# Livioni/OmniVGGT-official

Measured on AMD Instinct MI355X. Metric: frames/sec (518^2, S views) aggregator hot path, higher is better.
Workload: dtype bf16

## Files before the change

omnivggt-official_amd/csrc/ovg_gemm.hip:

```cpp
#include "ovg_common.h"
#include <mutex>
#include <type_traits>
#include <utility>
#include <vector>

namespace {

constexpr int BM = 128, BN = 128;

#ifdef OVG_GEMM_TIMELINE
__device__ unsigned long long* g_tl_buf = nullptr;
__device__ int g_tl_stagger = 0;
OVG_DEV void tl_mark(int slot) {
  if ((threadIdx.x & 63) != 0 || g_tl_buf == nullptr) return;
  const int wave = threadIdx.x >> 6, last = (blockDim.x >> 6) - 1;
  if (wave != 0 && wave != last) return;
  unsigned long long* row = g_tl_buf + (size_t)blockIdx.x * 16 + (wave == 0 ? 0 : 8);
  row[slot] = wall_clock64();
  if (slot == 0) { row[4] = __builtin_amdgcn_s_getreg((31 << 11) | 4); row[5] = __builtin_amdgcn_s_getreg((31 << 11) | 20); row[6] = clock64(); }
  if (slot == 3) row[7] = clock64();
}
OVG_DEV void tl_stagger() {
  if (g_tl_stagger <= 0 || blockIdx.x >= 256) return;
  const unsigned long long until = wall_clock64() + (unsigned long long)(((blockIdx.x >> 3) & 7) * g_tl_stagger);
  while (wall_clock64() < until) __builtin_amdgcn_s_sleep(16);
}
#else
OVG_DEV void tl_mark(int) {}
OVG_DEV void tl_stagger() {}
#endif

OVG_DEV float gelu_erf(float x) { return 0.5f * x * (1.0f + erff(x * 0.70710678118654752440f)); }
OVG_DEV void gelu_poly16(f32x4 (&v)[4]) {
  constexpr float c[13] = {1.413637876e-01f, -7.029628064e-02f, 5.152052248e-02f, -4.044260701e-02f, 3.144217031e-02f, -2.326865498e-02f,
                           1.640218381e-02f, -1.116433345e-02f, 6.410491046e-03f, -2.685581490e-03f, 1.722817794e-03f, -1.613262584e-03f,
                           6.087207876e-04f};
  f32x4 xc[4], u[4], r[4];
#pragma unroll
  for (int nt = 0; nt < 4; ++nt) {
#pragma unroll
    for (int i = 0; i < 4; ++i) xc[nt][i] = __builtin_amdgcn_fmed3f(v[nt][i], -5.0f, 5.0f);
    u[nt] = xc[nt] * xc[nt] * 0.08f - 1.0f;
    r[nt] = u[nt] * c[12] + c[11];
  }
#pragma unroll
  for (int k = 10; k >= 0; --k) {
#pragma unroll
    for (int nt = 0; nt < 4; ++nt) r[nt] = r[nt] * u[nt] + c[k];
  }
#pragma unroll
  for (int nt = 0; nt < 4; ++nt) v[nt] = v[nt] * (xc[nt] * r[nt] + 0.5f);
}

OVG_DEV void tile_coords(int lid, int mtiles, int ntiles_gm, int& tm, int& tn) {
  const int ntiles = ntiles_gm & 0xffff, GM = (ntiles_gm >> 16) & 0xff;
  if (GM == 0) { tm = lid / ntiles; tn = lid - tm * ntiles; return; }
  const int per_group = GM * ntiles;
  const int grp = lid / per_group, rem = lid - grp * per_group;
  const int m_first = grp * GM;
  const int gsz = (mtiles - m_first) < GM ? (mtiles - m_first) : GM;
  tm = m_first + rem % gsz;
  tn = rem / gsz;
}

template <typename T, bool SWAP = false, bool X3 = false>
OVG_DEV void gemm_mainloop(const T* __restrict__ X, int64_t ldx, const T* __restrict__ W, int64_t ldw,
                           int M, int N, int K, int m0, int n0, unsigned char* lds, f32x4 (&acc)[4][4],
                           const T* __restrict__ Xlo = nullptr, const T* __restrict__ Wlo = nullptr) {
  constexpr int BKB = 128;
  unsigned char* Ws = lds;
  unsigned char* Xs = lds + BN * BKB;
  const int tid = threadIdx.x, lane = tid & 63, wave = tid >> 6;
  const int wn = wave >> 1, wm = wave & 1;
  const int g = lane >> 4, lr = lane & 15;

  const unsigned char* xg[4];
  const unsigned char* wg[4];
  int soff[4];
#pragma unroll
  for (int i = 0; i < 4; ++i) {
    const int row = (tid >> 3) + 32 * i, ch = tid & 7;
    int xr = m0 + row; xr = xr < M ? xr : M - 1;
    int wr = n0 + row; wr = wr < N ? wr : N - 1;
    xg[i] = reinterpret_cast<const unsigned char*>(X + (int64_t)xr * ldx) + ch * 16;
    wg[i] = reinterpret_cast<const unsigned char*>(W + (int64_t)wr * ldw) + ch * 16;
// ... 59 lines not shown
        a[t] = *reinterpret_cast<const u32x4*>(Ws + wrow + t * 16 * 128 + coff);
        b[t] = *reinterpret_cast<const u32x4*>(Xs + xrow + t * 16 * 128 + coff);
      }
#pragma unroll
      for (int nt = 0; nt < 4; ++nt)
#pragma unroll
        for (int mt = 0; mt < 4; ++mt) {
          if constexpr (SWAP) TT<T>::mma(acc[nt][mt], b[mt], a[nt]);
          else TT<T>::mma(acc[nt][mt], a[nt], b[mt]);
        }
    }
    __syncthreads();
    if (more) {
#pragma unroll
      for (int i = 0; i < 4; ++i) {
        *reinterpret_cast<u32x4*>(Xs + soff[i]) = rx[i];
        *reinterpret_cast<u32x4*>(Ws + soff[i]) = rw[i];
      }
      __syncthreads();
    }
  }
}

template <typename T, int EPI, bool OUT_F32, int MT, bool INJECT, bool X3 = false>
OVG_DEV void linear_epilogue_impl(const ovg_linear_params& p, const f32x4 (&acc)[4][MT], const int m_w0, const int n_w0) {
  const int M = (int)p.M, N = (int)p.N;
  const int lane = threadIdx.x & 63, g = lane >> 4, lr = lane & 15;
  const int ncol = n_w0 + 4 * g;
  f32x4 bias[4], gam[4];
  if (p.bias != nullptr) {
#pragma unroll
    for (int nt = 0; nt < 4; ++nt) bias[nt] = *reinterpret_cast<const f32x4*>(p.bias + ncol + nt * 16);
  } else {
#pragma unroll
    for (int nt = 0; nt < 4; ++nt) bias[nt] = f32x4{0.f, 0.f, 0.f, 0.f};
  }
  if constexpr (EPI == OVG_EPI_RES) {
#pragma unroll
    for (int nt = 0; nt < 4; ++nt) gam[nt] = *reinterpret_cast<const f32x4*>(p.gamma + ncol + nt * 16);
  }
  constexpr bool kRowLoads = (EPI == OVG_EPI_RES || EPI == OVG_EPI_PATCH);
  constexpr int AH = !kRowLoads ? 0 : (MT == 8 ? 1 : 0);
  constexpr int NS = AH + 1;
  const FastDiv div_p0(EPI == OVG_EPI_PATCH ? (int)p.p0 : 1), div_per(INJECT ? (int)p.inj_period : 1);
  f32x4 ex[NS][4], inj[NS][4];
  float on[NS];
  int64_t orow_s[NS];
  auto fetch = [&](int mt, f32x4 (&exs)[4], f32x4 (&injs)[4], float& ons, int64_t& orow) {
    const int m = m_w0 + mt * 16 + lr;
    const int mc = m < M ? m : M - 1;
    orow = mc;
    ons = 0.f;
    if constexpr (EPI == OVG_EPI_PATCH) {
      int vw, t;
      div_p0.divmod(mc, vw, t);
      orow = (int64_t)vw * p.p1 + p.row_off + t;
      const float* trow = p.table + (int64_t)(t + 1) * N + ncol;
#pragma unroll
// ... 57 lines not shown
          store4_hilo(static_cast<f16_t*>(p.y) + off, static_cast<f16_t*>(p.y_lo) + off, v[nt][0], v[nt][1], v[nt][2], v[nt][3]);
        } else {
          store4<T>(static_cast<T*>(p.y) + orow * p.ldy + ncol + nt * 16, v[nt][0], v[nt][1], v[nt][2], v[nt][3]);
        }
      }
    }
  }
}

template <typename T> OVG_DEV void stage16_put4(unsigned char* img, int row, int col, float a, float b, float c, float d) {
  const int chunk = col >> 3, half = (col >> 2) & 1;
  store4<T>(reinterpret_cast<T*>(img + row * 128 + ((chunk ^ (row & 7)) << 4) + half * 8), a, b, c, d);
}
OVG_DEV u32x4 stage16_get(const unsigned char* img, int row, int chunk) {
  return *reinterpret_cast<const u32x4*>(img + row * 128 + ((chunk ^ (row & 7)) << 4));
}
OVG_DEV void stage32_put4(unsigned char* img, int row, int col, const f32x4 v) {
  *reinterpret_cast<f32x4*>(img + row * 256 + (((col >> 2) ^ (row & 15)) << 4)) = v;
}
OVG_DEV f32x4 stage32_get(const unsigned char* img, int row, int chunk) {
  return *reinterpret_cast<const f32x4*>(img + row * 256 + ((chunk ^ (row & 15)) << 4));
}

template <typename T, int EPI, int MT>
OVG_DEV void linear_epilogue_staged(const ovg_linear_params& p, const f32x4 (&acc)[4][MT], const int m_w0, const int n_w0, unsigned char* img) {
  const int M = (int)p.M;
  const int lane = threadIdx.x & 63, g = lane >> 4, lr = lane & 15;
  const int ncol = n_w0 + 4 * g;
  f32x4 bias[4];
  if (p.bias != nullptr) {
#pragma unroll
    for (int nt = 0; nt < 4; ++nt) bias[nt] = *reinterpret_cast<const f32x4*>(p.bias + ncol + nt * 16);
  } else {
#pragma unroll
    for (int nt = 0; nt < 4; ++nt) bias[nt] = f32x4{0.f, 0.f, 0.f, 0.f};
  }
  if constexpr (EPI == OVG_EPI_RES) {
    constexpr int HR = 8 * MT, HB = MT / 2, NI = HR / 4;
    f32x4 gam[4];
#pragma unroll
    for (int nt = 0; nt < 4; ++nt) {
      gam[nt] = *reinterpret_cast<const f32x4*>(p.gamma + ncol + nt * 16);
      bias[nt] = gam[nt] * bias[nt];
    }
    const int prow = lane >> 4, pch = lane & 15;
#pragma unroll
    for (int half = 0; half < 2; ++half) {
      f32x4 res[NI];
#pragma unroll
      for (int i = 0; i < NI; ++i) {
        int m = m_w0 + half * HR + i * 4 + prow;
        m = m < M ? m : M - 1;
        res[i] = *reinterpret_cast<const f32x4*>(p.res + (int64_t)m * p.ldres + n_w0 + pch * 4);
      }
#pragma unroll
      for (int ml = 0; ml < HB; ++ml)
#pragma unroll
        for (int nt = 0; nt < 4; ++nt) stage32_put4(img, ml * 16 + lr, nt * 16 + 4 * g, gam[nt] * acc[nt][half * HB + ml] + bias[nt]);
#pragma unroll
// ... 21 lines not shown
          for (int nt = 0; nt < 4; ++nt)
#pragma unroll
            for (int r = 0; r < 4; ++r) v[nt][r] = fminf(v[nt][r], 65504.0f);
        }
      }
#pragma unroll
      for (int nt = 0; nt < 4; ++nt) stage16_put4<T>(img, mt * 16 + lr, nt * 16 + 4 * g, v[nt][0], v[nt][1], v[nt][2], v[nt][3]);
    }
    const int prow = lane >> 3, pch = lane & 7;
#pragma unroll
    for (int i0 = 0; i0 < 2 * MT; i0 += 4) {
      u32x4 t[4];
#pragma unroll
      for (int j = 0; j < 4; ++j) t[j] = stage16_get(img, (i0 + j) * 8 + prow, pch);
#pragma unroll
      for (int j = 0; j < 4; ++j) {
        const int m = m_w0 + (i0 + j) * 8 + prow;
        if (m < M) *reinterpret_cast<u32x4*>(static_cast<T*>(p.y) + (int64_t)m * p.ldy + n_w0 + pch * 8) = t[j];
      }
    }
  }
}

template <typename T, int EPI, bool OUT_F32, int MT, bool X3 = false>
OVG_DEV void linear_epilogue(const ovg_linear_params& p, const f32x4 (&acc)[4][MT], const int m_w0, const int n_w0) {
  if constexpr (EPI == OVG_EPI_RES) {
    if (p.inject != nullptr) { linear_epilogue_impl<T, EPI, OUT_F32, MT, true, X3>(p, acc, m_w0, n_w0); return; }
  }
  linear_epilogue_impl<T, EPI, OUT_F32, MT, false, X3>(p, acc, m_w0, n_w0);
}

template <typename T, int EPI, bool OUT_F32, int MT, bool X3 = false>
OVG_DEV void linear_epilogue_auto(const ovg_linear_params& p, const f32x4 (&acc)[4][MT], const int m_w0, const int n_w0, unsigned char* img) {
  if constexpr (sizeof(T) == 2) {
    if constexpr ((EPI == OVG_EPI_STORE || EPI == OVG_EPI_GELU) && !OUT_F32 && !X3) {
      if (((p.ldy * (int64_t)sizeof(T)) & 15) == 0) { linear_epilogue_staged<T, EPI, MT>(p, acc, m_w0, n_w0, img); return; }
    }
    if constexpr (EPI == OVG_EPI_RES) {
      bool inj_here = false;
      if (p.inject != nullptr) {
        const int rem = m_w0 % (int)p.inj_period;
        inj_here = rem == 0 || (int)p.inj_period - rem < 16 * MT;
      }
      if (!inj_here) { linear_epilogue_staged<T, EPI, MT>(p, acc, m_w0, n_w0, img); return; }
    }
  }
  linear_epilogue<T, EPI, OUT_F32, MT, X3>(p, acc, m_w0, n_w0);
}


template <typename T, int EPI, bool OUT_F32, bool X3 = false>
__global__ __launch_bounds__(256, 2) void linear_kernel(ovg_linear_params p, int ntiles_n) {
  __shared__ __attribute__((aligned(16))) unsigned char lds[2 * 128 * 128];
  const int M = (int)p.M, N = (int)p.N, K = (int)p.K;
  int tm, tn;
  tl_stagger();
  tl_mark(0);
  tile_coords(xcd_remap(blockIdx.x, gridDim.x), (M + BM - 1) / BM, ntiles_n, tm, tn);
  const int m0 = tm * BM, n0 = tn * BN;
  f32x4 acc[4][4];
  gemm_mainloop<T, false, X3>(static_cast<const T*>(p.x), p.ldx, static_cast<const T*>(p.w), p.ldw, M, N, K, m0, n0, lds, acc,
                              static_cast<const T*>(p.x_lo), static_cast<const T*>(p.w_lo));
  tl_mark(2);
  const int wave = __builtin_amdgcn_readfirstlane(threadIdx.x >> 6);
  linear_epilogue_auto<T, EPI, OUT_F32, 4, X3>(p, acc, m0 + (wave & 1) * 64, n0 + (wave >> 1) * 64, lds + wave * 8192);
  tl_mark(3);
}

template <typename T, int MT, bool NORM, bool ROPE, bool X3 = false>
OVG_DEV void qk_rows(const f32x4 (&acc)[4][MT], const float* __restrict__ nw_p, const float* __restrict__ nb_p,
                     const float* __restrict__ rope_cos, const float* __restrict__ rope_sin, T* __restrict__ out, const int64_t npad,
                     const int m_w0, const int M, const int seq, const int h, const int tokens_per_view, const int n_special,
                     const int grid_w, const float qk_eps, const float scale, unsigned char* img = nullptr, T* __restrict__ out_lo = nullptr) {
  const int lane = threadIdx.x & 63, g = lane >> 4, lr = lane & 15;
  const FastDiv div_seq(seq), div_tpv(ROPE ? tokens_per_view : 1), div_gw(ROPE ? grid_w : 1);
  float nw[16], nb[16];
  if constexpr (NORM) {
#pragma unroll
    for (int nt = 0; nt < 4; ++nt) {
      const f32x4 a = *reinterpret_cast<const f32x4*>(nw_p + nt * 16 + 4 * g);
      const f32x4 b = *reinterpret_cast<const f32x4*>(nb_p + nt * 16 + 4 * g);
#pragma unroll
      for (int r = 0; r < 4; ++r) { nw[nt * 4 + r] = a[r]; nb[nt * 4 + r] = b[r]; }
    }
  }
#pragma unroll
  for (int mt = 0; mt < MT; ++mt) {
    const int m = m_w0 + mt * 16 + lr;
    const bool valid = m < M;
    const int mm = valid ? m : M - 1;
    int bidx, n;
    div_seq.divmod(mm, bidx, n);
    f32x4 cy, sy, cx, sxn;
    if constexpr (ROPE) {
      int vw, t, py, px;
      div_tpv.divmod(mm, vw, t);
      const int pp = t - n_special;
      div_gw.divmod(pp >= 0 ? pp : 0, py, px);
      py = pp >= 0 ? py + 1 : 0;
      px = pp >= 0 ? px + 1 : 0;
      cy = *reinterpret_cast<const f32x4*>(rope_cos + py * 16 + 4 * g);
      sy = *reinterpret_cast<const f32x4*>(rope_sin + py * 16 + 4 * g);
      cx = *reinterpret_cast<const f32x4*>(rope_cos + px * 16 + 4 * g);
      sxn = *reinterpret_cast<const f32x4*>(rope_sin + px * 16 + 4 * g);
    }
    float v[16];
#pragma unroll
    for (int nt = 0; nt < 4; ++nt)
// ... 45 lines not shown
      }
    }
  }
  if constexpr (sizeof(T) == 2) {
    if (img != nullptr) {
      const int prow = lane >> 3, pch = lane & 7;
#pragma unroll
      for (int i0 = 0; i0 < 2 * MT; i0 += 4) {
        u32x4 t[4];
#pragma unroll
        for (int j = 0; j < 4; ++j) t[j] = stage16_get(img, (i0 + j) * 8 + prow, pch);
#pragma unroll
        for (int j = 0; j < 4; ++j) {
          const int m = m_w0 + (i0 + j) * 8 + prow;
          int bidx, n;
          div_seq.divmod(m < M ? m : M - 1, bidx, n);
          if (m < M) *reinterpret_cast<u32x4*>(out + (((int64_t)bidx * OVG_H + h) * npad + n) * OVG_D + pch * 8) = t[j];
        }
      }
    }
  }
}

template <typename T, int MT, bool X3 = false>
OVG_DEV void qk_epilogue(const ovg_qkv_params& p, f32x4 (&acc)[4][MT], const int m_w0, const int ncol0_,
                         const float* rope_c, const float* rope_s, unsigned char* img = nullptr) {
  const int ncol0 = __builtin_amdgcn_readfirstlane(ncol0_);
  const int M = (int)p.M;
  const int lane = threadIdx.x & 63, g = lane >> 4;
  const int seq = (int)p.seq;
  const int which = ncol0 / OVG_C;
  const int h = (ncol0 % OVG_C) / OVG_D;

#pragma unroll
  for (int nt = 0; nt < 4; ++nt) {
    const f32x4 b = *reinterpret_cast<const f32x4*>(p.bias + ncol0 + nt * 16 + 4 * g);
#pragma unroll
    for (int mt = 0; mt < MT; ++mt) acc[nt][mt] += b;
  }
  {
    const float* nw_p = which == 0 ? p.qn_w : p.kn_w;
    const float* nb_p = which == 0 ? p.qn_b : p.kn_b;
    T* out = static_cast<T*>(which == 0 ? p.q : p.k);
    T* out_lo = static_cast<T*>(which == 0 ? p.q_lo : p.k_lo);
    const int64_t npad = which == 0 ? p.nq_pad : p.nk_pad;
    const float scale = which == 0 ? p.q_scale : 1.0f;
    const int tpv = (int)p.tokens_per_view;
#define OVG_QK_ROWS(NORM, ROPE) qk_rows<T, MT, NORM, ROPE, X3>(acc, nw_p, nb_p, rope_c, rope_s, out, npad, m_w0, M, seq, h, \
                                                                 tpv, p.n_special, p.grid_w, p.qk_eps, scale, img, out_lo)
    if (p.qk_norm) { if (p.rope) OVG_QK_ROWS(true, true); else OVG_QK_ROWS(true, false); }
    else { if (p.rope) OVG_QK_ROWS(false, true); else OVG_QK_ROWS(false, false); }
#undef OVG_QK_ROWS
  }
}

template <typename T, int MT, bool X3 = false>
OVG_DEV void v_epilogue(const ovg_qkv_params& p, const f32x4 (&acc)[4][MT], const int m_w0, const int ncol0_) {
  const int ncol0 = __builtin_amdgcn_readfirstlane(ncol0_);
  const int M = (int)p.M, seq = (int)p.seq;
  const int lane = threadIdx.x & 63, g = lane >> 4, lr = lane & 15;
  const int h = (ncol0 % OVG_C) / OVG_D;
  const FastDiv div_seq(seq);
  float bias[4];
#pragma unroll
  for (int nt = 0; nt < 4; ++nt) bias[nt] = p.bias[ncol0 + nt * 16 + lr];
  T* vt = static_cast<T*>(p.vt);
  const int64_t dlo = X3 ? static_cast<T*>(p.vt_lo) - vt : 0;
#pragma unroll
  for (int mt = 0; mt < MT; ++mt) {
    const int m = m_w0 + mt * 16 + 4 * g;
    const int mc = m < M ? m : M - 1;
    int bidx, n;
    div_seq.divmod(mc, bidx, n);
    const bool inside = (m + 3 < M) && (n + 3 < seq);
    const bool whole = inside && ((n & 3) == 0);
    const bool halves = sizeof(T) == 2 && inside && ((n & 3) == 2);
    T* rowb = vt + (((int64_t)bidx * OVG_H + h) * OVG_D + lr) * p.nk_pad;
    const int c0 = sizeof(T) == 2 ? vt_pos16(n) : n, c2 = sizeof(T) == 2 ? vt_pos16(n + 2) : n + 2;
#pragma unroll
    for (int nt = 0; nt < 4; ++nt) {
      const f32x4 v = acc[nt][mt] + bias[nt];
      T* dst = rowb + (int64_t)nt * 16 * p.nk_pad;
      if (whole) {
        if constexpr (X3) store4_hilo(dst + c0, dst + dlo + c0, v[0], v[1], v[2], v[3]);
        else store4<T>(dst + c0, v[0], v[1], v[2], v[3]);
      } else if (halves) {
        if constexpr (X3) {
          f16_t ph[4], pl[4];
// ... 57 lines not shown
  tl_stagger();
  tl_mark(0);
  tile_coords(xcd_remap(blockIdx.x, gridDim.x), (M + BM - 1) / BM, nt_count, tm, tn);
  const int m0 = tm * BM, n0 = (nt_begin + tn) * BN;
  const int wave = threadIdx.x >> 6;
  f32x4 acc[4][4];
  if (n0 >= 2 * OVG_C) {
    gemm_mainloop<T, true, X3>(static_cast<const T*>(p.x), p.ldx, static_cast<const T*>(p.w), (int64_t)K, M, N, K, m0, n0, lds, acc,
                               static_cast<const T*>(p.x_lo), static_cast<const T*>(p.w_lo));
    tl_mark(2);
    v_epilogue<T, 4, X3>(p, acc, m0 + (wave & 1) * 64, n0 + (wave >> 1) * 64);
  } else {
    gemm_mainloop<T, false, X3>(static_cast<const T*>(p.x), p.ldx, static_cast<const T*>(p.w), (int64_t)K, M, N, K, m0, n0, lds, acc,
                                static_cast<const T*>(p.x_lo), static_cast<const T*>(p.w_lo));
    tl_mark(2);
    unsigned char* img = (sizeof(T) == 2 && !X3) ? lds + __builtin_amdgcn_readfirstlane(wave) * 8192 : nullptr;
    qk_epilogue<T, 4, X3>(p, acc, m0 + (wave & 1) * 64, n0 + (wave >> 1) * 64, p.rope_cos, p.rope_sin, img);
  }
  tl_mark(3);
}

#include "ovg_gemm256.h"

template <typename T, int EPI, bool OUT_F32, bool X3 = false>
__global__ __launch_bounds__(512) void linear256_kernel(ovg_linear_params p, int ntiles_n) {
  extern __shared__ __attribute__((aligned(16))) unsigned char lds256[];
  const int M = (int)p.M, N = (int)p.N, K = (int)p.K;
  int tm, tn;
  tl_stagger();
  tl_mark(0);
  tile_coords(xcd_remap(blockIdx.x, gridDim.x), (M + g256::BM2 - 1) / g256::BM2, ntiles_n, tm, tn);
  const int m0 = tm * g256::BM2, n0 = tn * g256::BN2;
  f32x4 acc[4][8];
  g256::mainloop<T, false, X3>(static_cast<const T*>(p.x), p.ldx, static_cast<const T*>(p.w), p.ldw, M, N, K, m0, n0, lds256, acc,
                                static_cast<const T*>(p.x_lo), static_cast<const T*>(p.w_lo));
  tl_mark(2);
  const int wave = __builtin_amdgcn_readfirstlane(threadIdx.x >> 6);
  linear_epilogue_auto<T, EPI, OUT_F32, 8, X3>(p, acc, m0 + (wave >> 2) * 128, n0 + (wave & 3) * 64, lds256 + wave * 16384);
  tl_mark(3);
}

template <typename T, bool X3 = false>
__global__ __launch_bounds__(512) void qkv256_kernel(ovg_qkv_params p, int nt_begin, int nt_count) {
  extern __shared__ __attribute__((aligned(16))) unsigned char lds256[];
  constexpr int N = 3 * OVG_C, K = OVG_C;
  const int M = (int)p.M;
  int tm, tn;
  tl_stagger();
  tl_mark(0);
  tile_coords(xcd_remap(blockIdx.x, gridDim.x), (M + g256::BM2 - 1) / g256::BM2, nt_count, tm, tn);
  const int m0 = tm * g256::BM2, n0 = (nt_begin + tn) * g256::BN2;
  const int wave = threadIdx.x >> 6;
  f32x4 acc[4][8];
  if (n0 >= 2 * OVG_C) {
    g256::mainloop<T, true, X3>(static_cast<const T*>(p.x), p.ldx, static_cast<const T*>(p.w), (int64_t)K, M, N, K, m0, n0, lds256, acc,
                                 static_cast<const T*>(p.x_lo), static_cast<const T*>(p.w_lo));
    tl_mark(2);
    v_epilogue<T, 8, X3>(p, acc, m0 + (wave >> 2) * 128, n0 + (wave & 3) * 64);
  } else {
    float* rope_tab = reinterpret_cast<float*>(lds256 + g256::LDS_BYTES);
    stage_rope_table(p, lds256 + g256::LDS_BYTES, 8);
    g256::mainloop<T, false, X3>(static_cast<const T*>(p.x), p.ldx, static_cast<const T*>(p.w), (int64_t)K, M, N, K, m0, n0, lds256, acc,
                                  static_cast<const T*>(p.x_lo), static_cast<const T*>(p.w_lo));
    if constexpr (!X3) __builtin_amdgcn_sched_barrier(0);
    unsigned char* img = X3 ? nullptr : lds256 + __builtin_amdgcn_readfirstlane(wave) * 16384;
    tl_mark(2);
    qk_epilogue<T, 8, X3>(p, acc, m0 + (wave >> 2) * 128, n0 + (wave & 3) * 64, rope_tab, rope_tab + 128 * 16, img);
  }
  tl_mark(3);
}

template <typename KernelT>
int allow_big_lds(KernelT kernel, int bytes = g256::LDS_BYTES) {
  static std::mutex mu;
  static std::vector<std::pair<const void*, int>> done;
  const void* fn = reinterpret_cast<const void*>(kernel);
  int dev = 0;
  if (hipGetDevice(&dev) != hipSuccess) return OVG_E_LAUNCH;
  std::lock_guard<std::mutex> lock(mu);
  for (const auto& d : done)
    if (d.first == fn && d.second == dev) return OVG_OK;
  if (hipFuncSetAttribute(fn, hipFuncAttributeMaxDynamicSharedMemorySize, bytes) != hipSuccess) return OVG_E_LAUNCH;
  done.emplace_back(fn, dev);
  return OVG_OK;
}

constexpr int TILE_GROUP = 8, TILE_GROUP256 = 4;

bool aligned16(const void* p) { return (reinterpret_cast<uintptr_t>(p) & 15) == 0; }

template <typename T, int EPI, bool OUT_F32, bool X3>
int launch_linear_one(const ovg_linear_params& p, hipStream_t st, bool big) {
  if constexpr (sizeof(T) == 2) {
    if (big) {
      const int ok = allow_big_lds(linear256_kernel<T, EPI, OUT_F32, X3>);
      if (ok != OVG_OK) return ok;
      const int mt = (int)((p.M + g256::BM2 - 1) / g256::BM2), nt = (int)(p.N / g256::BN2);
      OVG_LAUNCH((linear256_kernel<T, EPI, OUT_F32, X3>), dim3(mt * nt), dim3(512), g256::LDS_BYTES, st, p, nt | (TILE_GROUP256 << 16));
      OVG_CHECK_LAUNCH();
      return OVG_OK;
    }
  }
  const int mt = (int)((p.M + BM - 1) / BM), nt = (int)(p.N / BN);
  OVG_LAUNCH((linear_kernel<T, EPI, OUT_F32, X3>), dim3(mt * nt), dim3(256), 0, st, p, nt | (TILE_GROUP << 16));
  OVG_CHECK_LAUNCH();
  return OVG_OK;
}
template <typename T, bool X3>
int dispatch_linear(const ovg_linear_params& p, hipStream_t st, bool big) {
  switch (p.epilogue) {
    case OVG_EPI_STORE: return p.out_f32 ? launch_linear_one<T, OVG_EPI_STORE, true, X3>(p, st, big) : launch_linear_one<T, OVG_EPI_STORE, false, X3>(p, st, big);
    case OVG_EPI_GELU: return launch_linear_one<T, OVG_EPI_GELU, false, X3>(p, st, big);
    case OVG_EPI_RES: return launch_linear_one<T, OVG_EPI_RES, true, X3>(p, st, big);
    case OVG_EPI_PATCH: return launch_linear_one<T, OVG_EPI_PATCH, true, X3>(p, st, big);
    default: return OVG_E_ARG;
  }
}
int gemm_device_cus() {
  static const int n = [] {
    int dev = 0, v = 0;
    if (hipGetDevice(&dev) != hipSuccess || hipDeviceGetAttribute(&v, hipDeviceAttributeMultiprocessorCount, dev) != hipSuccess || v <= 0) v = 256;
// ... 13 lines not shown
  if (kind == 2 && M >= 8000 && t256 <= cus) return 1;
  if (kind == 3 && t256 <= cus && t128 > 3 * cus) return 1;
  return 0;
}

template <typename T>
int launch_linear(const ovg_linear_params& p, hipStream_t st) {
  const int big = choose_256(p.tile, sizeof(T) == 2, p.M, p.N, p.K, p.epilogue != OVG_EPI_RES || p.K >= 2048,
                             p.epilogue == OVG_EPI_GELU ? 1 : (p.epilogue == OVG_EPI_RES ? (p.K >= 2048 ? 2 : 3) : 0));
  if (big < 0) return OVG_E_ARG;
  return dispatch_linear<T, false>(p, st, big != 0);
}

int launch_linear_x3(const ovg_linear_params& p, hipStream_t st) {
  const int big = choose_256(p.tile, true, p.M, p.N, p.K, true);
  if (big < 0) return OVG_E_ARG;
  return dispatch_linear<f16_t, true>(p, st, big != 0);
}

template <typename T, bool X3>
int launch_qkv(const ovg_qkv_params& p, hipStream_t st, bool big, int nt_begin, int nt_count) {
  if constexpr (sizeof(T) == 2) {
    if (big) {
      constexpr int lds_bytes = g256::LDS_BYTES + ROPE_LDS_BYTES;
      const int ok = allow_big_lds(qkv256_kernel<T, X3>, lds_bytes);
      if (ok != OVG_OK) return ok;
      const dim3 grid((unsigned)(((p.M + g256::BM2 - 1) / g256::BM2) * nt_count));
      OVG_LAUNCH((qkv256_kernel<T, X3>), grid, dim3(512), lds_bytes, st, p, nt_begin, nt_count | (TILE_GROUP256 << 16));
      OVG_CHECK_LAUNCH();
      return OVG_OK;
    }
  }
  const dim3 grid((unsigned)(((p.M + BM - 1) / BM) * nt_count));
  OVG_LAUNCH((qkv_kernel<T, X3>), grid, dim3(256), 0, st, p, nt_begin, nt_count | (TILE_GROUP << 16));
  OVG_CHECK_LAUNCH();
  return OVG_OK;
}

#ifdef OVG_GEMM_TIMELINE
}
extern "C" int ovg_lab_gemm_timeline(void* buf, int stagger_ticks) {
  unsigned long long* b = static_cast<unsigned long long*>(buf);
  if (hipMemcpyToSymbol(HIP_SYMBOL(g_tl_buf), &b, sizeof(b)) != hipSuccess) return OVG_E_LAUNCH;
  if (hipMemcpyToSymbol(HIP_SYMBOL(g_tl_stagger), &stagger_ticks, sizeof(int)) != hipSuccess) return OVG_E_LAUNCH;
  return OVG_OK;
}
namespace {
#endif

}

// ... 66 lines not shown
```

omnivggt-official_amd/csrc/ovg_gemm256.h:

```cpp
#pragma once

namespace g256 {

constexpr int BM2 = 256, BN2 = 256, ROWB = 64, SLOTS = 4;
constexpr int W_TILE = BN2 * ROWB, X_TILE = BM2 * ROWB, STAGE_B = W_TILE + X_TILE;
constexpr int LDS_BYTES = SLOTS * STAGE_B;
constexpr int NP = 4;

OVG_DEV int swz64(int row) { return (0x78 >> (2 * ((row >> 2) & 3))) & 3; }

OVG_DEV void wait_stages_in_flight(int n) {
  if (n >= 3) asm volatile("s_waitcnt vmcnt(12)" ::: "memory");
  else if (n == 2) asm volatile("s_waitcnt vmcnt(8)" ::: "memory");
  else if (n == 1) asm volatile("s_waitcnt vmcnt(4)" ::: "memory");
  else asm volatile("s_waitcnt vmcnt(0)" ::: "memory");
}

template <typename T, bool SWAP = false, bool X3 = false>
OVG_DEV void mainloop(const T* __restrict__ X, int64_t ldx, const T* __restrict__ W, int64_t ldw,
                      int M, int N, int K, int m0, int n0, unsigned char* lds, f32x4 (&acc)[4][8],
                      const T* __restrict__ Xlo = nullptr, const T* __restrict__ Wlo = nullptr) {
  static_assert(sizeof(T) == 2, "16-bit operands");
  const int tid = threadIdx.x, lane = tid & 63;
  const int wave = __builtin_amdgcn_readfirstlane(tid >> 6);
  const int wn = wave & 3, wm = wave >> 2;
  const int g = lane >> 4, lr = lane & 15;

  const unsigned char* wbase = reinterpret_cast<const unsigned char*>(W + (int64_t)n0 * ldw);
  const unsigned char* xbase = reinterpret_cast<const unsigned char*>(X + (int64_t)m0 * ldx);
  uint32_t wg[2], xg[2];
#pragma unroll
  for (int i = 0; i < 2; ++i) {
    const int row = wave * 32 + i * 16 + (lane >> 2);
    const int wr = n0 + row < N ? row : N - 1 - n0;
    const int xr = m0 + row < M ? row : M - 1 - m0;
    const uint32_t ch = (uint32_t)(((lane & 3) ^ swz64(row)) * 16);
    wg[i] = (uint32_t)wr * (uint32_t)(ldw * 2) + ch;
    xg[i] = (uint32_t)xr * (uint32_t)(ldx * 2) + ch;
  }
  const int nk1 = (K * 2) / ROWB;
  const int nk = X3 ? 3 * nk1 : nk1;
  const int64_t dxl = X3 ? reinterpret_cast<const unsigned char*>(Xlo) - reinterpret_cast<const unsigned char*>(X) : 0;
  const int64_t dwl = X3 ? reinterpret_cast<const unsigned char*>(Wlo) - reinterpret_cast<const unsigned char*>(W) : 0;
  const uint32_t lds_base = __builtin_amdgcn_readfirstlane((uint32_t)(uintptr_t)lds);
// ... 2 lines not shown
    int64_t xo = (int64_t)kt * ROWB, wo = xo;
    if constexpr (X3) {
      const int pass = kt >= 2 * nk1 ? 2 : (kt >= nk1 ? 1 : 0);
      const int64_t kb = (int64_t)(kt - pass * nk1) * ROWB;
      xo = kb + (pass == 0 ? dxl : 0);
      wo = kb + (pass == 1 ? dwl : 0);
    }
    if (j < 2) lds_dma16_s(wbase + wo, wg[j], sb + j * 16 * ROWB);
    else lds_dma16_s(xbase + xo, xg[j - 2], sb + W_TILE + (j - 2) * 16 * ROWB);
  };
#pragma unroll
  for (int a = 0; a < 4; ++a)
#pragma unroll
    for (int b = 0; b < 8; ++b) acc[a][b] = f32x4{0.f, 0.f, 0.f, 0.f};

  const int frag_off = lr * ROWB + (g ^ swz64(lr)) * 16;
  const unsigned char* wfrag = lds + wn * 64 * ROWB + frag_off;
  const unsigned char* xfrag = lds + W_TILE + wm * 128 * ROWB + frag_off;
  u32x4 a0[4], a1[4], b[8];

  for (int s = 0; s < SLOTS; ++s)
    if (s < nk)
      for (int j = 0; j < NP; ++j) stage_piece(s, j);
  wait_stages_in_flight((nk < SLOTS ? nk : SLOTS) - 1);
  __builtin_amdgcn_s_barrier();
  tl_mark(1);
#pragma unroll
  for (int t = 0; t < 4; ++t) a0[t] = *reinterpret_cast<const u32x4*>(wfrag + t * 16 * ROWB);
#pragma unroll
  for (int t = 0; t < 8; ++t) b[t] = *reinterpret_cast<const u32x4*>(xfrag + t * 16 * ROWB);

  auto body = [&](int t, const u32x4 (&acur)[4], u32x4 (&anxt)[4], bool dma, int infl) __attribute__((always_inline)) {
    asm volatile("s_waitcnt lgkmcnt(0)" ::: "memory");
    if (infl >= 0) wait_stages_in_flight(infl);
    __builtin_amdgcn_s_barrier();
    __builtin_amdgcn_sched_barrier(0);
    const int so = ((t + 1) & (SLOTS - 1)) * STAGE_B;
    const unsigned char* wn_ = wfrag + so;
    const unsigned char* xn_ = xfrag + so;
#pragma unroll
    for (int mt = 0; mt < 8; ++mt) {
#pragma unroll
      for (int nt = 0; nt < 4; ++nt) {
        if constexpr (SWAP) TT<T>::mma(acc[nt][mt], b[mt], acur[nt]);
        else TT<T>::mma(acc[nt][mt], acur[nt], b[mt]);
      }
// ... 23 lines not shown
```

Before: 81.76.

## Prefetch successor tiles' X panels into L2 during GEMM epilogues

Adds a cross-block L2 warming scheme to the 256-tile linear and QKV kernels. Each block works out which block will run on its XCD after it, and whether that block will be the first to use a new X row panel. If so, it issues global_load_lds_dword touches into a small dummy LDS area during its epilogue, or right after the first mainloop loads, so the successor's cold misses are paid early. This adds extra memory traffic, LDS use and scheduling assumptions about XCD round-robin residency, which may not match the real dispatch order.

```diff
diff --git a/omnivggt-official_amd/csrc/ovg_gemm.hip b/omnivggt-official_amd/csrc/ovg_gemm.hip
--- a/omnivggt-official_amd/csrc/ovg_gemm.hip
+++ b/omnivggt-official_amd/csrc/ovg_gemm.hip
@@ -1,4 +1,5 @@
 #include "ovg_common.h"
+#include "ovg_gemm_warm.h"
 #include <mutex>
 #include <type_traits>
 #include <utility>
@@ -20,6 +21,19 @@
   if (slot == 0) { row[4] = __builtin_amdgcn_s_getreg((31 << 11) | 4); row[5] = __builtin_amdgcn_s_getreg((31 << 11) | 20); row[6] = clock64(); }
   if (slot == 3) row[7] = clock64();
 }
+OVG_DEV void tl_tile(int lid, int tm, int tn, int mtiles, int packed) {
+  if (g_tl_buf == nullptr || threadIdx.x != blockDim.x - 64) return;
+  const int ntiles = packed & 0xffff, gm = (packed >> 16) & 0xff, resident = (packed >> 24) & 0x7f;
+  int first = 0;
+  if (gm > 0 && resident > 0) {
+    int start, count, ptm, n, r;
+    ovg_warm::xcd_run(blockIdx.x & 7, gridDim.x, start, count);
+    first = ovg_warm::panel_first_use(lid, start, start + count, resident, mtiles, ntiles, gm, ptm, n, r) ? 1 : 0;
+  }
+  unsigned long long* row = g_tl_buf + (size_t)blockIdx.x * 16 + 8;
+  row[4] = (unsigned long long)(unsigned)lid | ((unsigned long long)first << 32);
+  row[5] = (unsigned long long)(unsigned)tn | ((unsigned long long)(unsigned)tm << 32);
+}
 OVG_DEV void tl_stagger() {
   if (g_tl_stagger <= 0 || blockIdx.x >= 256) return;
   const unsigned long long until = wall_clock64() + (unsigned long long)(((blockIdx.x >> 3) & 7) * g_tl_stagger);
@@ -27,6 +41,7 @@
 }
 #else
 OVG_DEV void tl_mark(int) {}
+OVG_DEV void tl_tile(int, int, int, int, int) {}
 OVG_DEV void tl_stagger() {}
 #endif
 
@@ -53,14 +68,49 @@
 }
 
 OVG_DEV void tile_coords(int lid, int mtiles, int ntiles_gm, int& tm, int& tn) {
-  const int ntiles = ntiles_gm & 0xffff, GM = (ntiles_gm >> 16) & 0xff;
-  if (GM == 0) { tm = lid / ntiles; tn = lid - tm * ntiles; return; }
-  const int per_group = GM * ntiles;
-  const int grp = lid / per_group, rem = lid - grp * per_group;
-  const int m_first = grp * GM;
-  const int gsz = (mtiles - m_first) < GM ? (mtiles - m_first) : GM;
-  tm = m_first + rem % gsz;
-  tn = rem / gsz;
+  ovg_warm::tile_of(lid, mtiles, ntiles_gm & 0xffff, (ntiles_gm >> 16) & 0xff, tm, tn);
+}
+
+constexpr int WARM_LDS_BYTES = 256;
+#ifndef OVG_GEMM_WARM
+#define OVG_GEMM_WARM 1
+#endif
+struct NoWarm {
+  static constexpr bool enabled = false;
+  OVG_DEV void issue() const {}
+};
+struct Warm {
+  static constexpr bool enabled = true;
+  const unsigned char* x;
+  uint32_t ldb;
+  uint32_t dump;
+  ovg_warm::Plan plan;
+  OVG_DEV void pin() { asm volatile("" : "+s"(plan.row0), "+s"(plan.rows), "+s"(plan.bytes), "+s"(dump)); }
+  OVG_DEV void issue() const {
+    if (plan.rows <= 0) return;
+    const int shift = ovg_warm::line_shift(plan);
+    const int n = ovg_warm::passes(plan, shift, 9);
+    const unsigned char* sbase = x + (int64_t)plan.row0 * ldb;
+    for (int pass = 0; pass < n; ++pass) {
+      int row, col;
+      if (ovg_warm::touch(plan, shift, 9, (int)threadIdx.x, pass, row, col)) {
+        const uint32_t voff = (uint32_t)(row - plan.row0) * ldb + (uint32_t)col;
+        asm volatile("s_mov_b32 m0, %0\n\ts_nop 0\n\tglobal_load_lds_dword %1, %2" ::"s"(dump), "v"(voff), "s"(sbase) : "memory");
+      }
+    }
+  }
+};
+template <typename V> OVG_DEV void landed(const V& a, const V& b, const V& c, const V& d) { asm volatile("" ::"v"(a), "v"(b), "v"(c), "v"(d)); }
+template <typename T>
+OVG_DEV Warm make_warm(const T* x, int64_t ldx, int M, int K, int lid, int mtiles, int packed, unsigned char* dump) {
+  Warm w;
+  w.x = reinterpret_cast<const unsigned char*>(x);
+  w.ldb = (uint32_t)(ldx * (int64_t)sizeof(T));
+  w.dump = __builtin_amdgcn_readfirstlane((uint32_t)(uintptr_t)dump);
+  int start, count;
+  ovg_warm::xcd_run(blockIdx.x & 7, gridDim.x, start, count);
+  w.plan = ovg_warm::plan_in_run(lid, start, count, mtiles, packed & 0xffff, (packed >> 16) & 0xff, (packed >> 24) & 0x7f, M, K, ldx, (int)sizeof(T));
+  return w;
 }
 
 template <typename T, bool SWAP = false, bool X3 = false>
@@ -166,8 +216,8 @@
   }
 }
 
-template <typename T, int EPI, bool OUT_F32, int MT, bool INJECT, bool X3 = false>
-OVG_DEV void linear_epilogue_impl(const ovg_linear_params& p, const f32x4 (&acc)[4][MT], const int m_w0, const int n_w0) {
+template <typename T, int EPI, bool OUT_F32, int MT, bool INJECT, bool X3 = false, class W = NoWarm>
+OVG_DEV void linear_epilogue_impl(const ovg_linear_params& p, const f32x4 (&acc)[4][MT], const int m_w0, const int n_w0, const W& warm = W()) {
   const int M = (int)p.M, N = (int)p.N;
   const int lane = threadIdx.x & 63, g = lane >> 4, lr = lane & 15;
   const int ncol = n_w0 + 4 * g;
@@ -178,6 +228,11 @@
   } else {
 #pragma unroll
     for (int nt = 0; nt < 4; ++nt) bias[nt] = f32x4{0.f, 0.f, 0.f, 0.f};
+  }
+  if constexpr (W::enabled) {
+    static_assert(EPI == OVG_EPI_STORE || EPI == OVG_EPI_GELU, "the row-loading epilogues have waits of their own");
+    landed(bias[0], bias[1], bias[2], bias[3]);
+    warm.issue();
   }
   if constexpr (EPI == OVG_EPI_RES) {
 #pragma unroll
@@ -281,8 +336,9 @@
   return *reinterpret_cast<const f32x4*>(img + row * 256 + ((chunk ^ (row & 15)) << 4));
 }
 
-template <typename T, int EPI, int MT>
-OVG_DEV void linear_epilogue_staged(const ovg_linear_params& p, const f32x4 (&acc)[4][MT], const int m_w0, const int n_w0, unsigned char* img) {
+template <typename T, int EPI, int MT, class W = NoWarm>
+OVG_DEV void linear_epilogue_staged(const ovg_linear_params& p, const f32x4 (&acc)[4][MT], const int m_w0, const int n_w0, unsigned char* img,
+                                    const W& warm = W()) {
   const int M = (int)p.M;
   const int lane = threadIdx.x & 63, g = lane >> 4, lr = lane & 15;
   const int ncol = n_w0 + 4 * g;
@@ -294,6 +350,11 @@
 #pragma unroll
     for (int nt = 0; nt < 4; ++nt) bias[nt] = f32x4{0.f, 0.f, 0.f, 0.f};
   }
+  if constexpr (W::enabled) {
+    static_assert(EPI == OVG_EPI_STORE || EPI == OVG_EPI_GELU, "the residual epilogue has waits of its own");
+    landed(bias[0], bias[1], bias[2], bias[3]);
+    warm.issue();
+  }
   if constexpr (EPI == OVG_EPI_RES) {
     constexpr int HR = 8 * MT, HB = MT / 2, NI = HR / 4;
     f32x4 gam[4];
@@ -361,19 +422,20 @@
   }
 }
 
-template <typename T, int EPI, bool OUT_F32, int MT, bool X3 = false>
-OVG_DEV void linear_epilogue(const ovg_linear_params& p, const f32x4 (&acc)[4][MT], const int m_w0, const int n_w0) {
+template <typename T, int EPI, bool OUT_F32, int MT, bool X3 = false, class W = NoWarm>
+OVG_DEV void linear_epilogue(const ovg_linear_params& p, const f32x4 (&acc)[4][MT], const int m_w0, const int n_w0, const W& warm = W()) {
   if constexpr (EPI == OVG_EPI_RES) {
     if (p.inject != nullptr) { linear_epilogue_impl<T, EPI, OUT_F32, MT, true, X3>(p, acc, m_w0, n_w0); return; }
   }
-  linear_epilogue_impl<T, EPI, OUT_F32, MT, false, X3>(p, acc, m_w0, n_w0);
-}
-
-template <typename T, int EPI, bool OUT_F32, int MT, bool X3 = false>
-OVG_DEV void linear_epilogue_auto(const ovg_linear_params& p, const f32x4 (&acc)[4][MT], const int m_w0, const int n_w0, unsigned char* img) {
+  linear_epilogue_impl<T, EPI, OUT_F32, MT, false, X3, W>(p, acc, m_w0, n_w0, warm);
+}
+
+template <typename T, int EPI, bool OUT_F32, int MT, bool X3 = false, class W = NoWarm>
+OVG_DEV void linear_epilogue_auto(const ovg_linear_params& p, const f32x4 (&acc)[4][MT], const int m_w0, const int n_w0, unsigned char* img,
+                                  const W& warm = W()) {
   if constexpr (sizeof(T) == 2) {
     if constexpr ((EPI == OVG_EPI_STORE || EPI == OVG_EPI_GELU) && !OUT_F32 && !X3) {
-      if (((p.ldy * (int64_t)sizeof(T)) & 15) == 0) { linear_epilogue_staged<T, EPI, MT>(p, acc, m_w0, n_w0, img); return; }
+      if (((p.ldy * (int64_t)sizeof(T)) & 15) == 0) { linear_epilogue_staged<T, EPI, MT, W>(p, acc, m_w0, n_w0, img, warm); return; }
     }
     if constexpr (EPI == OVG_EPI_RES) {
       bool inj_here = false;
@@ -384,7 +446,7 @@
       if (!inj_here) { linear_epilogue_staged<T, EPI, MT>(p, acc, m_w0, n_w0, img); return; }
     }
   }
-  linear_epilogue<T, EPI, OUT_F32, MT, X3>(p, acc, m_w0, n_w0);
+  linear_epilogue<T, EPI, OUT_F32, MT, X3, W>(p, acc, m_w0, n_w0, warm);
 }
 
 
@@ -406,23 +468,29 @@
   tl_mark(3);
 }
 
-template <typename T, int MT, bool NORM, bool ROPE, bool X3 = false>
+template <typename T, int MT, bool NORM, bool ROPE, bool X3 = false, class W = NoWarm>
 OVG_DEV void qk_rows(const f32x4 (&acc)[4][MT], const float* __restrict__ nw_p, const float* __restrict__ nb_p,
                      const float* __restrict__ rope_cos, const float* __restrict__ rope_sin, T* __restrict__ out, const int64_t npad,
                      const int m_w0, const int M, const int seq, const int h, const int tokens_per_view, const int n_special,
-                     const int grid_w, const float qk_eps, const float scale, unsigned char* img = nullptr, T* __restrict__ out_lo = nullptr) {
+                     const int grid_w, const float qk_eps, const float scale, unsigned char* img = nullptr, T* __restrict__ out_lo = nullptr,
+                     const W& warm = W()) {
   const int lane = threadIdx.x & 63, g = lane >> 4, lr = lane & 15;
   const FastDiv div_seq(seq), div_tpv(ROPE ? tokens_per_view : 1), div_gw(ROPE ? grid_w : 1);
   float nw[16], nb[16];
   if constexpr (NORM) {
+    f32x4 a[4], b[4];
 #pragma unroll
     for (int nt = 0; nt < 4; ++nt) {
-      const f32x4 a = *reinterpret_cast<const f32x4*>(nw_p + nt * 16 + 4 * g);
-      const f32x4 b = *reinterpret_cast<const f32x4*>(nb_p + nt * 16 + 4 * g);
-#pragma unroll
-      for (int r = 0; r < 4; ++r) { nw[nt * 4 + r] = a[r]; nb[nt * 4 + r] = b[r]; }
-    }
-  }
+      a[nt] = *reinterpret_cast<const f32x4*>(nw_p + nt * 16 + 4 * g);
+      b[nt] = *reinterpret_cast<const f32x4*>(nb_p + nt * 16 + 4 * g);
+    }
+    if constexpr (W::enabled) { landed(a[0], a[1], a[2], a[3]); landed(b[0], b[1], b[2], b[3]); }
+#pragma unroll
+    for (int nt = 0; nt < 4; ++nt)
+#pragma unroll
+      for (int r = 0; r < 4; ++r) { nw[nt * 4 + r] = a[nt][r]; nb[nt * 4 + r] = b[nt][r]; }
+  }
+  warm.issue();
 #pragma unroll
   for (int mt = 0; mt < MT; ++mt) {
     const int m = m_w0 + mt * 16 + lr;
@@ -514,9 +582,9 @@
   }
 }
 
-template <typename T, int MT, bool X3 = false>
+template <typename T, int MT, bool X3 = false, class W = NoWarm>
 OVG_DEV void qk_epilogue(const ovg_qkv_params& p, f32x4 (&acc)[4][MT], const int m_w0, const int ncol0_,
-                         const float* rope_c, const float* rope_s, unsigned char* img = nullptr) {
+                         const float* rope_c, const float* rope_s, unsigned char* img = nullptr, const W& warm = W()) {
   const int ncol0 = __builtin_amdgcn_readfirstlane(ncol0_);
   const int M = (int)p.M;
   const int lane = threadIdx.x & 63, g = lane >> 4;
@@ -524,12 +592,14 @@
   const int which = ncol0 / OVG_C;
   const int h = (ncol0 % OVG_C) / OVG_D;
 
-#pragma unroll
-  for (int nt = 0; nt < 4; ++nt) {
-    const f32x4 b = *reinterpret_cast<const f32x4*>(p.bias + ncol0 + nt * 16 + 4 * g);
-#pragma unroll
-    for (int mt = 0; mt < MT; ++mt) acc[nt][mt] += b;
-  }
+  f32x4 b[4];
+#pragma unroll
+  for (int nt = 0; nt < 4; ++nt) b[nt] = *reinterpret_cast<const f32x4*>(p.bias + ncol0 + nt * 16 + 4 * g);
+  if constexpr (W::enabled) landed(b[0], b[1], b[2], b[3]);
+#pragma unroll
+  for (int nt = 0; nt < 4; ++nt)
+#pragma unroll
+    for (int mt = 0; mt < MT; ++mt) acc[nt][mt] += b[nt];
   {
     const float* nw_p = which == 0 ? p.qn_w : p.kn_w;
     const float* nb_p = which == 0 ? p.qn_b : p.kn_b;
@@ -538,16 +608,16 @@
     const int64_t npad = which == 0 ? p.nq_pad : p.nk_pad;
     const float scale = which == 0 ? p.q_scale : 1.0f;
     const int tpv = (int)p.tokens_per_view;
-#define OVG_QK_ROWS(NORM, ROPE) qk_rows<T, MT, NORM, ROPE, X3>(acc, nw_p, nb_p, rope_c, rope_s, out, npad, m_w0, M, seq, h, \
-                                                                 tpv, p.n_special, p.grid_w, p.qk_eps, scale, img, out_lo)
+#define OVG_QK_ROWS(NORM, ROPE) qk_rows<T, MT, NORM, ROPE, X3, W>(acc, nw_p, nb_p, rope_c, rope_s, out, npad, m_w0, M, seq, h, \
+                                                                    tpv, p.n_special, p.grid_w, p.qk_eps, scale, img, out_lo, warm)
     if (p.qk_norm) { if (p.rope) OVG_QK_ROWS(true, true); else OVG_QK_ROWS(true, false); }
     else { if (p.rope) OVG_QK_ROWS(false, true); else OVG_QK_ROWS(false, false); }
 #undef OVG_QK_ROWS
   }
 }
 
-template <typename T, int MT, bool X3 = false>
-OVG_DEV void v_epilogue(const ovg_qkv_params& p, const f32x4 (&acc)[4][MT], const int m_w0, const int ncol0_) {
+template <typename T, int MT, bool X3 = false, class W = NoWarm>
+OVG_DEV void v_epilogue(const ovg_qkv_params& p, const f32x4 (&acc)[4][MT], const int m_w0, const int ncol0_, const W& warm = W()) {
   const int ncol0 = __builtin_amdgcn_readfirstlane(ncol0_);
   const int M = (int)p.M, seq = (int)p.seq;
   const int lane = threadIdx.x & 63, g = lane >> 4, lr = lane & 15;
@@ -556,6 +626,7 @@
   float bias[4];
 #pragma unroll
   for (int nt = 0; nt < 4; ++nt) bias[nt] = p.bias[ncol0 + nt * 16 + lr];
+  if constexpr (W::enabled) { landed(bias[0], bias[1], bias[2], bias[3]); warm.issue(); }
   T* vt = static_cast<T*>(p.vt);
   const int64_t dlo = X3 ? static_cast<T*>(p.vt_lo) - vt : 0;
 #pragma unroll
@@ -659,6 +730,7 @@
 
 #include "ovg_gemm256.h"
 
+template <int EPI, bool X3> constexpr bool kWarm256 = OVG_GEMM_WARM && !X3 && (EPI == OVG_EPI_STORE || EPI == OVG_EPI_GELU);
 template <typename T, int EPI, bool OUT_F32, bool X3 = false>
 __global__ __launch_bounds__(512) void linear256_kernel(ovg_linear_params p, int ntiles_n) {
   extern __shared__ __attribute__((aligned(16))) unsigned char lds256[];
@@ -666,14 +738,24 @@
   int tm, tn;
   tl_stagger();
   tl_mark(0);
-  tile_coords(xcd_remap(blockIdx.x, gridDim.x), (M + g256::BM2 - 1) / g256::BM2, ntiles_n, tm, tn);
+  const int lid = xcd_remap(blockIdx.x, gridDim.x), mtiles = (M + g256::BM2 - 1) / g256::BM2;
+  tile_coords(lid, mtiles, ntiles_n, tm, tn);
+  tl_tile(lid, tm, tn, mtiles, ntiles_n);
   const int m0 = tm * g256::BM2, n0 = tn * g256::BN2;
   f32x4 acc[4][8];
+  using W = typename std::conditional<kWarm256<EPI, X3>, Warm, NoWarm>::type;
+  W warm;
+  auto plan_warm = [&]() {
+    if constexpr (W::enabled) {
+      warm = make_warm(static_cast<const T*>(p.x), p.ldx, M, K, lid, mtiles, ntiles_n, lds256 + g256::LDS_BYTES);
+      warm.pin();
+    }
+  };
   g256::mainloop<T, false, X3>(static_cast<const T*>(p.x), p.ldx, static_cast<const T*>(p.w), p.ldw, M, N, K, m0, n0, lds256, acc,
-                                static_cast<const T*>(p.x_lo), static_cast<const T*>(p.w_lo));
+                                static_cast<const T*>(p.x_lo), static_cast<const T*>(p.w_lo), plan_warm);
   tl_mark(2);
   const int wave = __builtin_amdgcn_readfirstlane(threadIdx.x >> 6);
-  linear_epilogue_auto<T, EPI, OUT_F32, 8, X3>(p, acc, m0 + (wave >> 2) * 128, n0 + (wave & 3) * 64, lds256 + wave * 16384);
+  linear_epilogue_auto<T, EPI, OUT_F32, 8, X3, W>(p, acc, m0 + (wave >> 2) * 128, n0 + (wave & 3) * 64, lds256 + wave * 16384, warm);
   tl_mark(3);
 }
 
@@ -685,30 +767,41 @@
   int tm, tn;
   tl_stagger();
   tl_mark(0);
-  tile_coords(xcd_remap(blockIdx.x, gridDim.x), (M + g256::BM2 - 1) / g256::BM2, nt_count, tm, tn);
+  const int lid = xcd_remap(blockIdx.x, gridDim.x), mtiles = (M + g256::BM2 - 1) / g256::BM2;
+  tile_coords(lid, mtiles, nt_count, tm, tn);
+  tl_tile(lid, tm, tn, mtiles, nt_count);
   const int m0 = tm * g256::BM2, n0 = (nt_begin + tn) * g256::BN2;
   const int wave = threadIdx.x >> 6;
+  constexpr bool kWarm = OVG_GEMM_WARM && !X3;
+  using W = typename std::conditional<kWarm, Warm, NoWarm>::type;
+  W warm;
+  auto plan_warm = [&]() {
+    if constexpr (kWarm) {
+      warm = make_warm(static_cast<const T*>(p.x), p.ldx, M, K, lid, mtiles, nt_count, lds256 + g256::LDS_BYTES + ROPE_LDS_BYTES);
+      warm.pin();
+    }
+  };
   f32x4 acc[4][8];
   if (n0 >= 2 * OVG_C) {
     g256::mainloop<T, true, X3>(static_cast<const T*>(p.x), p.ldx, static_cast<const T*>(p.w), (int64_t)K, M, N, K, m0, n0, lds256, acc,
-                                 static_cast<const T*>(p.x_lo), static_cast<const T*>(p.w_lo));
+                                 static_cast<const T*>(p.x_lo), static_cast<const T*>(p.w_lo), plan_warm);
     tl_mark(2);
-    v_epilogue<T, 8, X3>(p, acc, m0 + (wave >> 2) * 128, n0 + (wave & 3) * 64);
+    v_epilogue<T, 8, X3, W>(p, acc, m0 + (wave >> 2) * 128, n0 + (wave & 3) * 64, warm);
   } else {
     float* rope_tab = reinterpret_cast<float*>(lds256 + g256::LDS_BYTES);
     stage_rope_table(p, lds256 + g256::LDS_BYTES, 8);
     g256::mainloop<T, false, X3>(static_cast<const T*>(p.x), p.ldx, static_cast<const T*>(p.w), (int64_t)K, M, N, K, m0, n0, lds256, acc,
-                                  static_cast<const T*>(p.x_lo), static_cast<const T*>(p.w_lo));
+                                  static_cast<const T*>(p.x_lo), static_cast<const T*>(p.w_lo), plan_warm);
     if constexpr (!X3) __builtin_amdgcn_sched_barrier(0);
     unsigned char* img = X3 ? nullptr : lds256 + __builtin_amdgcn_readfirstlane(wave) * 16384;
     tl_mark(2);
-    qk_epilogue<T, 8, X3>(p, acc, m0 + (wave >> 2) * 128, n0 + (wave & 3) * 64, rope_tab, rope_tab + 128 * 16, img);
+    qk_epilogue<T, 8, X3, W>(p, acc, m0 + (wave >> 2) * 128, n0 + (wave & 3) * 64, rope_tab, rope_tab + 128 * 16, img, warm);
   }
   tl_mark(3);
 }
 
 template <typename KernelT>
-int allow_big_lds(KernelT kernel, int bytes = g256::LDS_BYTES) {
+int allow_big_lds(KernelT kernel, int bytes) {
   static std::mutex mu;
   static std::vector<std::pair<const void*, int>> done;
   const void* fn = reinterpret_cast<const void*>(kernel);
@@ -724,16 +817,20 @@
 
 constexpr int TILE_GROUP = 8, TILE_GROUP256 = 4;
 
+int gemm_device_cus();
+int resident_per_xcd() { const int r = gemm_device_cus() / 8; return r < 1 ? 1 : (r > 127 ? 127 : r); }
+
 bool aligned16(const void* p) { return (reinterpret_cast<uintptr_t>(p) & 15) == 0; }
 
 template <typename T, int EPI, bool OUT_F32, bool X3>
 int launch_linear_one(const ovg_linear_params& p, hipStream_t st, bool big) {
   if constexpr (sizeof(T) == 2) {
     if (big) {
-      const int ok = allow_big_lds(linear256_kernel<T, EPI, OUT_F32, X3>);
+      constexpr int lds_bytes = g256::LDS_BYTES + (kWarm256<EPI, X3> ? WARM_LDS_BYTES : 0);
+      const int ok = allow_big_lds(linear256_kernel<T, EPI, OUT_F32, X3>, lds_bytes);
       if (ok != OVG_OK) return ok;
       const int mt = (int)((p.M + g256::BM2 - 1) / g256::BM2), nt = (int)(p.N / g256::BN2);
-      OVG_LAUNCH((linear256_kernel<T, EPI, OUT_F32, X3>), dim3(mt * nt), dim3(512), g256::LDS_BYTES, st, p, nt | (TILE_GROUP256 << 16));
+      OVG_LAUNCH((linear256_kernel<T, EPI, OUT_F32, X3>), dim3(mt * nt), dim3(512), lds_bytes, st, p, nt | (TILE_GROUP256 << 16) | (resident_per_xcd() << 24));
       OVG_CHECK_LAUNCH();
       return OVG_OK;
     }
@@ -793,11 +890,11 @@
 int launch_qkv(const ovg_qkv_params& p, hipStream_t st, bool big, int nt_begin, int nt_count) {
   if constexpr (sizeof(T) == 2) {
     if (big) {
-      constexpr int lds_bytes = g256::LDS_BYTES + ROPE_LDS_BYTES;
+      constexpr int lds_bytes = g256::LDS_BYTES + ROPE_LDS_BYTES + WARM_LDS_BYTES;
       const int ok = allow_big_lds(qkv256_kernel<T, X3>, lds_bytes);
       if (ok != OVG_OK) return ok;
       const dim3 grid((unsigned)(((p.M + g256::BM2 - 1) / g256::BM2) * nt_count));
-      OVG_LAUNCH((qkv256_kernel<T, X3>), grid, dim3(512), lds_bytes, st, p, nt_begin, nt_count | (TILE_GROUP256 << 16));
+      OVG_LAUNCH((qkv256_kernel<T, X3>), grid, dim3(512), lds_bytes, st, p, nt_begin, nt_count | (TILE_GROUP256 << 16) | (resident_per_xcd() << 24));
       OVG_CHECK_LAUNCH();
       return OVG_OK;
     }
diff --git a/omnivggt-official_amd/csrc/ovg_gemm256.h b/omnivggt-official_amd/csrc/ovg_gemm256.h
--- a/omnivggt-official_amd/csrc/ovg_gemm256.h
+++ b/omnivggt-official_amd/csrc/ovg_gemm256.h
@@ -16,10 +16,11 @@
   else asm volatile("s_waitcnt vmcnt(0)" ::: "memory");
 }
 
-template <typename T, bool SWAP = false, bool X3 = false>
+struct NoHook { OVG_DEV void operator()() const {} };
+template <typename T, bool SWAP = false, bool X3 = false, class Hook = NoHook>
 OVG_DEV void mainloop(const T* __restrict__ X, int64_t ldx, const T* __restrict__ W, int64_t ldw,
                       int M, int N, int K, int m0, int n0, unsigned char* lds, f32x4 (&acc)[4][8],
-                      const T* __restrict__ Xlo = nullptr, const T* __restrict__ Wlo = nullptr) {
+                      const T* __restrict__ Xlo = nullptr, const T* __restrict__ Wlo = nullptr, const Hook& under_first_loads = Hook()) {
   static_assert(sizeof(T) == 2, "16-bit operands");
   const int tid = threadIdx.x, lane = tid & 63;
   const int wave = __builtin_amdgcn_readfirstlane(tid >> 6);
@@ -68,6 +69,7 @@
   for (int s = 0; s < SLOTS; ++s)
     if (s < nk)
       for (int j = 0; j < NP; ++j) stage_piece(s, j);
+  under_first_loads();
   wait_stages_in_flight((nk < SLOTS ? nk : SLOTS) - 1);
   __builtin_amdgcn_s_barrier();
   tl_mark(1);
diff --git a/omnivggt-official_amd/csrc/ovg_gemm_warm.h b/omnivggt-official_amd/csrc/ovg_gemm_warm.h
--- /dev/null
+++ b/omnivggt-official_amd/csrc/ovg_gemm_warm.h
@@ -0,0 +1,96 @@
+#pragma once
+#include <cstdint>
+
+#if defined(__HIPCC__)
+#define OVG_WARM_FN __host__ __device__ inline
+#else
+#define OVG_WARM_FN inline
+#endif
+
+namespace ovg_warm {
+
+constexpr int TILE_ROWS = 256;
+constexpr int LINE = 128;
+
+OVG_WARM_FN void tile_of(int lid, int mtiles, int ntiles, int gm, int& tm, int& tn) {
+  if (gm == 0) { tm = lid / ntiles; tn = lid - tm * ntiles; return; }
+  const int per_group = gm * ntiles;
+  const int grp = lid / per_group, rem = lid - grp * per_group;
+  const int m_first = grp * gm;
+  const int gsz = (mtiles - m_first) < gm ? (mtiles - m_first) : gm;
+  tm = m_first + rem % gsz;
+  tn = rem / gsz;
+}
+
+OVG_WARM_FN void xcd_run(int x, int grid, int& start, int& count) {
+  const int q = grid >> 3, r = grid & 7;
+  start = x < r ? x * (q + 1) : r * (q + 1) + (x - r) * q;
+  count = q + (x < r ? 1 : 0);
+}
+OVG_WARM_FN int xcd_of(int lid, int grid) {
+  const int q = grid >> 3, r = grid & 7, big = r * (q + 1);
+  return lid < big ? lid / (q + 1) : r + (lid - big) / q;
+}
+
+OVG_WARM_FN int count_below(int x, int d, int c) { return x <= c ? 0 : (x - c + d - 1) / d; }
+
+OVG_WARM_FN bool panel_first_use(int lid, int run_start, int run_end, int resident, int mtiles, int ntiles, int gm, int& tm, int& sharers, int& rank) {
+  const int per_group = gm * ntiles;
+  const int grp = lid / per_group, gstart = grp * per_group;
+  const int m_first = grp * gm;
+  const int gsz = (mtiles - m_first) < gm ? (mtiles - m_first) : gm;
+  const int rem = lid - gstart, c = rem % gsz;
+  tm = m_first + c;
+  const int rb = run_start + (lid - run_start) / resident * resident;
+  const int re = rb + resident < run_end ? rb + resident : run_end;
+  const int gend = gstart + gsz * ntiles;
+  const int before = (run_start > gstart ? run_start : gstart) - gstart;
+  const int lo = (rb > gstart ? rb : gstart) - gstart;
+  const int hi = (re < gend ? re : gend) - gstart;
+  const int below_lo = count_below(lo, gsz, c);
+  sharers = count_below(hi, gsz, c) - below_lo;
+  rank = count_below(rem, gsz, c) - below_lo;
+  return below_lo == count_below(before, gsz, c);
+}
+
+struct Plan { int row0, rows, col0, bytes; };
+
+OVG_WARM_FN Plan plan_in_run(int lid, int run_start, int run_count, int mtiles, int ntiles, int gm, int resident, int M, int K, int64_t ldx, int esz) {
+  const Plan none = {0, 0, 0, 0};
+  if (gm <= 0 || resident <= 0) return none;
+  if ((int64_t)TILE_ROWS * ldx * esz >= ((int64_t)1 << 31) || (int64_t)K * esz > 512 * LINE) return none;
+  const int succ = lid + resident;
+  if (succ >= run_start + run_count) return none;
+  int tm, n, r;
+  if (!panel_first_use(succ, run_start, run_start + run_count, resident, mtiles, ntiles, gm, tm, n, r)) return none;
+  const int row0 = tm * TILE_ROWS;
+  const int rows = M - row0 < TILE_ROWS ? M - row0 : TILE_ROWS;
+  const int r0 = rows * r / n, r1 = rows * (r + 1) / n;
+  if (r1 <= r0) return none;
+  const Plan p = {row0 + r0, r1 - r0, 0, K * esz};
+  return p;
+}
+OVG_WARM_FN Plan plan(int lid, int grid, int mtiles, int ntiles, int gm, int resident, int M, int K, int64_t ldx, int esz) {
+  const Plan none = {0, 0, 0, 0};
+  if (lid < 0 || lid >= grid) return none;
+  int run_start, run_count;
+  xcd_run(xcd_of(lid, grid), grid, run_start, run_count);
+  return plan_in_run(lid, run_start, run_count, mtiles, ntiles, gm, resident, M, K, ldx, esz);
+}
+
+OVG_WARM_FN int line_shift(const Plan& p) {
+  const int lines = (p.bytes + LINE - 1) / LINE;
+  int s = 0;
+  while ((1 << s) < lines) ++s;
+  return s;
+}
+OVG_WARM_FN int passes(const Plan& p, int shift, int lg) { return (p.rows + (1 << (lg - shift)) - 1) >> (lg - shift); }
+OVG_WARM_FN bool touch(const Plan& p, int shift, int lg, int t, int pass, int& row, int& col) {
+  const int line = t & ((1 << shift) - 1);
+  const int ri = (t >> shift) + (pass << (lg - shift));
+  row = p.row0 + ri;
+  col = p.col0 + line * LINE;
+  return ri < p.rows && line * LINE < p.bytes;
+}
+
+}
```

Result: no change. 82.32 (median of 6 runs) (+0.7%).
